# GadGadGad/Convolutional-KAN-for-Image-Classification

Measured on AMD Instinct MI355X. Metric: images/sec fwd+bwd KAN-VGG11 3x32x32 bs=256/GPU, higher is better.
Workload: dtype f32

## Files before the change

### convolutional-kan-for-image-classification_amd/_lib.py

```python
from __future__ import annotations

import ctypes as C
import os
from typing import Optional

_HERE = os.path.dirname(os.path.abspath(__file__))
LIB_PATH = os.environ.get("KANCONV_LIB") or os.path.join(_HERE, "libkanconv.so")

KAN_MAX_PLANES = 16
KAN_MAX_TABLE = 32
KAN_FP_WORDS = 192
BASIS_BSPLINE, BASIS_RBF, BASIS_CHEBY, BASIS_POLY, BASIS_FOURIER, BASIS_RELU, BASIS_GRAM = 0, 1, 2, 3, 4, 5, 6
ACT_NONE, ACT_IDENTITY, ACT_GELU, ACT_SILU, ACT_RELU, ACT_TANH, ACT_SIGMOID, ACT_GELU_TANH = -1, 0, 1, 2, 3, 4, 5, 6
ORDER_QUAD_FWD, ORDER_ROWBLK8_FWD, ORDER_QUAD_BWD_DATA, ORDER_FWD_WEIGHT_SIDE = 1, 2, 4, 8


class KanGeom(C.Structure):
    _fields_ = [(n, C.c_int) for n in ("B", "C", "H", "W", "O", "Ho", "Wo", "kh", "kw", "sh", "sw", "ph", "pw", "dh", "dw", "groups")] + \
               [("x_bstride", C.c_longlong), ("y_bstride", C.c_longlong)]


class KanBasis(C.Structure):
    _fields_ = [("kind", C.c_int), ("n_basis", C.c_int), ("order", C.c_int), ("act", C.c_int),
                ("p0", C.c_float), ("p1", C.c_float), ("table", C.c_float * KAN_MAX_TABLE), ("chan_table", C.c_void_p)]


class KanPlan(C.Structure):
    _fields_ = [(n, C.c_int) for n in ("P", "K", "IPC", "KC", "Kpad", "Opad", "fwd_splits", "bwd_data_splits", "bwd_weight_splits",
                                          "fwd_target", "bwd_data_target", "bwd_weight_target", "x_pm_wanted", "dz_pm_wanted", "bwd_weight_expanded", "row_blocks", "e_pm_wanted", "fwd_expanded", "fwd_halo", "bwd_weight_halo",
# ... 31 lines not shown
_GP, _BP = C.POINTER(KanGeom), C.POINTER(KanBasis)
SIGNATURES = {
    "kan_version": (C.c_char_p, []),
    "kan_last_error": (C.c_char_p, []),
    "kan_plan": (_I, [_GP, _BP, C.POINTER(KanPlan)]),
    "kan_tile_orders": (_I, [_GP, _BP]),
    "kan_pack_weights": (_I, [_P, _P, _P, _P, _GP, _BP, _P]),
    "kan_pack_weights_iod": (_I, [_P, _P, _P, _GP, _BP, _P]),
    "kan_pack_cacheable": (_I, [_GP, _BP]),
    "kan_pack_weights_cached": (_I, [_P, _P, _P, _P, _GP, _BP, _P, _I, _I, _I, _P]),
    "kan_conv_fwd": (_I, [_P, _P, _P, _P, _GP, _BP, _P, _P]),
    "kan_position_major": (_I, [_P, _P, _I, _I, _I, _LL, _P]),
    "kan_conv_bwd_data": (_I, [_P, _P, _P, _P, _P, _P, _GP, _BP, _P, _P]),
    "kan_conv_bwd_data_params": (_I, [_P, _P, _P, _P, _P, _P, _P, _GP, _BP, _P, _P]),
    "kan_conv_bwd_weight": (_I, [_P, _P, _P, _P, _GP, _BP, _P, _P, _P]),
    "kan_position_major_expanded": (_I, [_P, _P, _GP, _BP, _P]),
    "kan_conv_fwd_expanded": (_I, [_P, _P, _P, _GP, _BP, _P]),
    "kan_conv_fwd_expanded_order": (_I, [_P, _P, _P, _GP, _BP, _P, _I]),
    "kan_conv_bwd_weight_expanded": (_I, [_P, _P, _P, _GP, _BP, _P]),
    "kan_unpack_wgrad": (_I, [_P, _P, _P, _GP, _BP, _P]),
    "kan_unpack_wgrad_iod": (_I, [_P, _P, _GP, _BP, _P]),
    "kan_slab_reduce": (_I, [_P, _I, _LL, _P, _I, _I, _I, _LL, _P]),
    "kan_instnorm_prelu_fwd": (_I, [_P, _I, _LL, _P, _P, _P, _P, _P, _P, _P, _I, _I, _I, _LL, _F, _I, _P]),
    "kan_instnorm_prelu_bwd": (_I, [_P, _P, _P, _P, _P, _P, _P, _P, _P, _P, _P, _I, _I, _I, _LL, _I, _P]),
    "kan_instnorm_prelu_pool_fwd": (_I, [_P, _I, _LL, _P, _P, _P, _P, _P, _P, _P, _P, _I, _I, _I, _I, _LL, _F, _I, _P]),
    "kan_instnorm_prelu_pool_bwd": (_I, [_P, _P, _P, _P, _P, _P, _P, _P, _P, _P, _P, _P, _I, _I, _I, _I, _LL, _I, _P]),
    "kan_instnorm_prelu_poolk_fwd": (_I, [_P, _I, _LL, _P, _P, _P, _P, _P, _P, _P, _P, _I, _I, _I, _I, _LL, _F, _I, _I, _I, _P]),
    "kan_instnorm_prelu_poolk_bwd": (_I, [_P, _P, _P, _P, _P, _P, _P, _P, _P, _P, _P, _P, _I, _I, _I, _I, _LL, _I, _I, _I, _P]),
    "kan_norm_route": (_I, [_I, _I, _I, _I, _I, _LL, _I, _LL, _I, _I, _I, _I, C.POINTER(KanNormRoute)]),
    "kan_batchnorm_workspace_bytes": (_LL, [_I, _I]),
# ... 60 lines not shown
```

### convolutional-kan-for-image-classification_amd/csrc/kan_internal.h

```cpp
#pragma once
#include <type_traits>
#include "kanconv.h"

int kan_fail_msg(const char* fmt, const char* a);
int kan_raise_lds_limit(const void* kernel, int bytes);

enum : int {
    FAST_GENERIC = 0,
    FAST_BSPLINE_SILU = 1,
    FAST_BSPLINE_GELU = 2,
    FAST_RBF8 = 3,
    FAST_CHEBY5 = 4,
    FAST_CHEBY4 = 5,
    FAST_POLY4 = 6,
    FAST_POLY3 = 7,
    FAST_RBF5 = 8,
    FAST_RELU8 = 9,
    FAST_GRAM4 = 10,
    FAST_POLY1 = 11,
    FAST_LAST = 11
};
enum : unsigned {
    ON_TAP_MAJOR = 1u << 0,
    ON_BIG_TILES = 1u << 1,
// ... 93 lines not shown

struct FwdCfg { int TO, TP, tiles_o, tiles_p, chunks, splits, slots; };
struct BdCfg { int CH, tiles_c, tiles_p, n_ob, Opad32, chunks, splits; };
struct BwCfg { int TR, TO, tiles_r, tiles_o, chunks, splits, slots; };
struct BwHaloCfg { int R, nimg, spb, n_bands, tiles_r, tiles_o, splits, bands_per_split; };

struct ConvPlan {
    KanPlan pub;
    int fast;
    Route fwd, bwd_data, bwd_weight;
    bool pm_fwd, pm_bwd_data, pm_bwd_weight;
    bool rowblk_bwd_data;
    bool quad_fwd;
    bool quad_bd;
    bool rowblk8_fwd;
    bool fwd_wq;
    bool pmdma_xcd, pm_lpt, pm_xcd;
    FwdCfg fc;
    BdCfg bd;
    BwCfg bw;
    BwHaloCfg bwh;
    KanBandCfg band;
};
int plan_conv(const KanGeom* g, const KanBasis* b, ConvPlan* cp);

int live_taps_out(const KanGeom* g, int hw);
int live_taps_in(const KanGeom* g, int hw);
int live_positions_for_tap(const KanGeom* g, int tap);
int balance_tiles(const int* weight, int n, unsigned short* idx);
```

### convolutional-kan-for-image-classification_amd/csrc/kan_plan.hip

```cpp
#include <hip/hip_runtime.h>
#include <cstdio>
#include <cstdlib>
#include <cstring>
#include "kanconv.h"
#include "kan_device.h"
#include "kan_common.h"
#include "kan_internal.h"

namespace {

int fail(const char* msg) { return kan_fail_msg("%s", msg); }

int check(const KanGeom* g, const KanBasis* b) {
    if (!g || !b) return fail("null geometry/basis");
    if (g->groups < 0 || g->groups > 65535) return fail("groups out of range");
    if (g->B <= 0 || g->C <= 0 || g->O <= 0 || g->H <= 0 || g->W <= 0 || g->Ho <= 0 || g->Wo <= 0) return fail("non-positive dimension");
    if (g->kh <= 0 || g->kw <= 0 || g->sh <= 0 || g->sw <= 0 || g->dh <= 0 || g->dw <= 0 || g->ph < 0 || g->pw < 0) return fail("bad conv parameters");
    if (g->kh > 255 || g->kw > 255 || g->C > 65535) return fail("kernel size / channel count out of supported range");
    if ((g->H + 2 * g->ph - g->dh * (g->kh - 1) - 1) / g->sh + 1 != g->Ho || (g->W + 2 * g->pw - g->dw * (g->kw - 1) - 1) / g->sw + 1 != g->Wo)
        return fail("Ho/Wo inconsistent with H/W, kernel, stride, padding, dilation");
    if ((long long)g->B * g->Ho * g->Wo >= (1ll << 31) || (long long)g->B * g->H * g->W >= (1ll << 31)) return fail("pixel count exceeds int32");
    if ((long long)g->B * g->x_bstride * 4 >= (1ll << 31) || (long long)g->B * g->y_bstride * 4 >= (1ll << 31))
        return fail("activation tensors must be smaller than 2 GiB (32-bit buffer offsets)");
    if (g->x_bstride < (long long)ngroups(g) * g->C * g->H * g->W || g->y_bstride < (long long)ngroups(g) * g->O * g->Ho * g->Wo)
// ... 326 lines not shown
    c.fc = fwd_cfg(g, *pl, big, c.pm_fwd, halo);
    c.bw = bw_cfg(g, *pl, big, c.pm_bwd_weight);
    if (halo_bw) c.bwh = bw_halo_cfg(g, *pl);
    pl->fwd_splits = band ? c.band.fwd_splits : c.fc.splits;
    pl->bwd_data_splits = c.bd.splits;
    pl->bwd_weight_splits = halo_bw ? c.bwh.splits : c.bw.splits;
    if (band_bw) {
        pl->bwd_weight_splits = c.band.bw_splits;
        pl->bwd_weight_slab_elems = (long long)G * pl->Kpad * pl->Opad;
    }
    pl->fwd_target = pl->bwd_data_target = pl->bwd_weight_target = 0;
    const bool rowblk_fwd = halo && g->H == 4 && g->W == 4 && c.fc.TO == 256;
    c.quad_fwd = rowblk_fwd && g->B % 32 == 0 && !tuning_off("KAN_QUAD_FWD");
    c.quad_bd = c.rowblk_bwd_data && g->B % 32 == 0 && !tuning_off("KAN_QUAD_BD");
    c.rowblk8_fwd = halo && g->H == 8 && g->W == 8 && c.fc.TO == 256 && g->B % 4 == 0 && !tuning_off("KAN_ROWBLK8_FWD");
    c.fwd_wq = c.fwd == Route::EXPANDED && g->H == 2 && g->W == 2 && g->Ho == 2 && g->Wo == 2 && g->kh == 3 && g->kw == 3 && g->sh == 1 && g->sw == 1 &&
               g->ph == 1 && g->pw == 1 && g->dh == 1 && g->dw == 1 && pl->P == 9 && pl->KC == 18 && g->y_bstride % 4 == 0 && !tuning_off("KAN_PMDMA_FWD_WQ");
    if (dw) {
        pl->fwd_splits = pl->bwd_data_splits = 1;
        pl->bwd_weight_splits = dw_weight_chunks(g);
        pl->bwd_data_weight_bytes = pl->packed_weight_bytes;
        c.pm_fwd = c.pm_bwd_data = c.pm_bwd_weight = false;
    }
    if (c.pm_fwd) {
        LiveClass cls[16]; const int plane = g->Ho * g->Wo;
        const long long tiles_per_pos = (long long)ceil_div(g->B, c.fc.TP) * c.fc.tiles_o * G;
        for (int hw = 0; hw < plane; ++hw) cls[hw] = LiveClass{tiles_per_pos, live_taps_out(g, hw) * ceil_div(g->C, pl->IPC)};
        pl->fwd_target = pick_target_steps(cls, plane, 8, 4.0 * g->B * g->O * g->Ho * g->Wo * G, &pl->fwd_splits, c.fc.slots);
    }
    if (c.pm_bwd_weight) {
// ... 25 lines not shown
```

### convolutional-kan-for-image-classification_amd/csrc/kanconv.hip

```cpp
#include <hip/hip_runtime.h>
#include <cstdio>
#include <cstdlib>
#include <cstring>
#include <cmath>
#include <cstdint>
#include <mutex>
#include <type_traits>
#include <vector>
#include "kanconv.h"
#include "kan_device.h"

#include "kan_common.h"
#include "kan_internal.h"

namespace {


thread_local char g_err[512] = "";
int fail(const char* fmt, const char* a = "") {
    snprintf(g_err, sizeof(g_err), fmt, a);
    return -1;
}
}
int kan_fail_msg(const char* fmt, const char* a) { return fail(fmt, a); }
// ... 1296 lines not shown
        for (int r = 0; r < 16; ++r) {
            const int row = k0 + w_r * 64 + mi * 32 + mfma_row(r, lane);
            if (row >= Krows) continue;
#pragma unroll
            for (int ni = 0; ni < 2; ++ni) {
                const int o = o_tile0 + w_c * 64 + ni * 32 + (lane & 31);
                out[(size_t)row * Opad + o] = acc[mi][ni][r];
            }
        }
}

#define LDS_READ4W(r0, r1, r2, r3, a0, a1, b, oA, oB0, oB1)                                                              \
    asm volatile("ds_read_b32 %0, %4 offset:%7\n\tds_read_b32 %1, %5 offset:%7\n\tds_read_b32 %2, %6 offset:%8\n\tds_read_b32 %3, %6 offset:%9" \
                 : "=&v"(r0), "=&v"(r1), "=&v"(r2), "=&v"(r3) : "v"(a0), "v"(a1), "v"(b), "n"(oA), "n"(oB0), "n"(oB1) : "memory")

template <int FAST, int W, int R, int NIMG>
__global__ __launch_bounds__(256, 4) void k_conv_bwd_weight_halo(
    const float* __restrict__ dz, const float* __restrict__ x, float* __restrict__ dwp, DevGeom g, DevBasis bs, int Krows, int Opad,
    int n_bands, int bands_per_split, long long slab_elems, unsigned x_bytes, unsigned dz_bytes, int tiles_o) {
    constexpr int KIND = fast_kind(FAST);
    constexpr int P = fast_planes(FAST), T = 9, PT = P * T;
    constexpr int TR = 128, TO = 128, NT = 256, KPX = 16;
    constexpr int HWc = W + 2, HIMG = (R + 2) * HWc, CELLS = NIMG * HIMG;
    constexpr int PS = W == 16 ? CELLS + 1 : W == 8 ? CELLS + 3 : W == 4 ? CELLS + 7 : CELLS + 1;
    constexpr int NCH = (TR + PT - 2) / PT + 1;
    constexpr int HB = NCH * P * PS;
    constexpr int BP = NIMG * R * W, SPB = BP / KPX;
    constexpr int ZB = KPX * TO;
    constexpr int NU = NCH * NIMG * (R + 2) * W;
    constexpr int SLOTS = (NU + NT - 1) / NT;
    static_assert(BP % KPX == 0 && SPB % 2 == 0 && SPB >= SLOTS + 1 && PS > CELLS && (NIMG == 1 || R == W), "band shape");
    __shared__ float sH[2 * HB];
    __shared__ __attribute__((aligned(16))) float sZ[2 * ZB];
    __shared__ float sTab[KAN_MAX_TABLE];

    const int tid = threadIdx.x, lane = tid & 63;
    const int wave = __builtin_amdgcn_readfirstlane(tid >> 6);
    const int w_r = wave >> 1, w_c = wave & 1, kh2 = lane >> 5;
    const int HoWo = g.Ho * g.Wo, HW = g.H * g.W;
    const BlockId blk = xcd_block_order(true);
    const int grp = blk.y / tiles_o;
    const int k0 = blk.x * TR, o_tile0 = (blk.y - grp * tiles_o) * TO;
    x += (size_t)grp * g.C * HW;
    dz += (size_t)grp * g.O * HoWo;
    dwp += (size_t)grp * Krows * Opad;
    const int c0 = k0 / PT;

    if (tid < KAN_MAX_TABLE) sTab[tid] = bs.tab[tid];
    for (int i = tid; i < 2 * HB; i += NT) sH[i] = 0.f;
    float* const dump = sH + CELLS;

    int u_src[SLOTS], u_dst[SLOTS], u_hr[SLOTS], u_ch[SLOTS]; unsigned u_ok = 0;
#pragma unroll
    for (int k = 0; k < SLOTS; ++k) {
        const int idx = tid + k * NT;
        constexpr int UPC = NIMG * (R + 2) * W, UPI = (R + 2) * W;
        const int ch = idx / UPC, ri = idx - ch * UPC, img = ri / UPI, rc = ri - img * UPI, hr = rc / W, col = rc - hr * W;
        u_src[k] = (c0 + ch) * HW + img * (int)g.xbs + (hr - 1) * W + col;
        u_dst[k] = ch * (P * PS) + img * HIMG + hr * HWc + col + 1;
        u_hr[k] = hr - 1; u_ch[k] = c0 + ch;
        u_ok |= ((idx < NU && c0 + ch < g.C) ? 1u : 0u) << k;
    }
    const kan_rsrc x_rs = make_rsrc(x, x_bytes), dz_rs = make_rsrc(dz, dz_bytes);

    unsigned aA[2];
#pragma unroll
    for (int mi = 0; mi < 2; ++mi) {
        int row = k0 + w_r * 64 + mi * 32 + (lane & 31);
        if (row >= Krows) row = k0;
        const int c = row / PT, rem = row - c * PT, tap = rem / P, pl_ = rem - tap * P, r = tap / 3, t = tap - 3 * r;
        aA[mi] = lds_addr(sH + ((c - c0) * P + pl_) * PS + r * HWc + t + kh2);
    }
    unsigned bB[KPX / 2];
    {
        const int ol = w_c * 64 + (lane & 31), sw = (ol >> 1) & 15;
#pragma unroll
        for (int kk = 0; kk < KPX / 2; ++kk) bB[kk] = lds_addr(sZ + ol * KPX + ((2 * kk + kh2) ^ sw));
    }
    unsigned zoff[8];
#pragma unroll
    for (int j = 0; j < 8; ++j) {
        const int ol = 4 * (wave * 8 + j) + (lane >> 4), q = (lane & 15) ^ ((ol >> 1) & 15);
        zoff[j] = o_tile0 + ol < g.O ? (unsigned)((o_tile0 + ol) * HoWo + q) * 4u : KAN_OOB;
    }
    constexpr int BPI = NIMG > 1 ? 1 : (W * W) / BP;
    auto issue_dz = [&](int band, int st, int zb) {
        const int gpx = band * BP + st * KPX;
        const int b = gpx / (W * W), px0 = gpx - b * (W * W);
        const int soff = __builtin_amdgcn_readfirstlane((b * (int)g.ybs + px0) * 4);
        float* dst = sZ + zb * ZB + wave * (8 * 64);
#pragma unroll
        for (int j = 0; j < 8; ++j)
            __builtin_amdgcn_raw_ptr_buffer_load_lds(dz_rs, (__attribute__((address_space(3))) void*)(dst + j * 64), 4, (int)zoff[j], soff, 0, 0);
    };
    float xv[SLOTS]; unsigned inb_mask = 0;
    auto load_band = [&](int band) {
        const int b = NIMG > 1 ? band * NIMG : band / BPI, h0 = NIMG > 1 ? 0 : (band - b * BPI) * R;
        const int sbase = b * (int)g.xbs + h0 * W;
        inb_mask = 0;
#pragma unroll
        for (int k = 0; k < SLOTS; ++k) {
            const bool inb = ((u_ok >> k) & 1u) && (unsigned)(h0 + u_hr[k]) < (unsigned)g.H;
            xv[k] = buf_load(x_rs, inb ? (unsigned)(sbase + u_src[k]) * 4u : KAN_OOB);
            inb_mask |= (inb ? 1u : 0u) << k;
        }
// ... 22 lines not shown
    int hb = 0;
    for (int band = nb0; band < nb1; ++band, hb ^= 1) {
        const unsigned hoff = (unsigned)(hb * HB * 4);
        const unsigned a0 = aA[0] + hoff, a1 = aA[1] + hoff;
#pragma unroll
        for (int st = 0; st < SPB; ++st) {
            asm volatile("s_waitcnt vmcnt(0)" ::: "memory");
            __syncthreads();
            if (st + 1 < SPB) issue_dz(band, st + 1, (st + 1) & 1);
            else if (band + 1 < nb1) issue_dz(band + 1, 0, 0);
            if (st == 0) { if (band + 1 < nb1) load_band(band + 1); }
            else if (st - 1 < SLOTS) { if (band + 1 < nb1) expand(st - 1, hb ^ 1); }
            float fa[2][2], fb[2][2];
#define KAN_OFFA(kk) ((((16 * st + 2 * (kk)) / (R * W)) * HIMG + (((16 * st + 2 * (kk)) % (R * W)) / W) * HWc + ((16 * st + 2 * (kk)) % W)) * 4)
#define KAN_OFFB(kk) (((st & 1) * ZB) * 4)
            LDS_READ4W(fa[0][0], fa[0][1], fb[0][0], fb[0][1], a0, a1, bB[0], KAN_OFFA(0), KAN_OFFB(0), KAN_OFFB(0) + 32 * KPX * 4);
#pragma unroll
            for (int kk = 0; kk < KPX / 2; ++kk) {
                const int c_ = kk & 1, n_ = c_ ^ 1;
                if (kk + 1 < KPX / 2) {
                    LDS_READ4W(fa[n_][0], fa[n_][1], fb[n_][0], fb[n_][1], a0, a1, bB[kk + 1], KAN_OFFA(kk + 1), KAN_OFFB(kk + 1),
                               KAN_OFFB(kk + 1) + 32 * KPX * 4);
                    LDS_WAIT4(fa[c_][0], fa[c_][1], fb[c_][0], fb[c_][1], 4);
                } else {
                    LDS_WAIT4(fa[c_][0], fa[c_][1], fb[c_][0], fb[c_][1], 0);
                }
                acc[0][0] = MFMA32(fa[c_][0], fb[c_][0], acc[0][0]);
                acc[0][1] = MFMA32(fa[c_][0], fb[c_][1], acc[0][1]);
                acc[1][0] = MFMA32(fa[c_][1], fb[c_][0], acc[1][0]);
                acc[1][1] = MFMA32(fa[c_][1], fb[c_][1], acc[1][1]);
            }
#undef KAN_OFFA
#undef KAN_OFFB
        }
    }

    float* out = dwp + (size_t)blk.z * slab_elems;
#pragma unroll
    for (int mi = 0; mi < 2; ++mi)
#pragma unroll
        for (int r = 0; r < 16; ++r) {
            const int row = k0 + w_r * 64 + mi * 32 + mfma_row(r, lane);
            if (row >= Krows) continue;
#pragma unroll
            for (int ni = 0; ni < 2; ++ni) {
                const int o = o_tile0 + w_c * 64 + ni * 32 + (lane & 31);
                out[(size_t)row * Opad + o] = acc[mi][ni][r];
            }
        }
}

template <int KIND, int FAST>
__global__ __launch_bounds__(256) void k_expand_pm(const float* __restrict__ x, float* __restrict__ e_pm, DevBasis bs, int B, int CHW, int HW, int Cg,
                                                   long long bstride, float* __restrict__ dump) {
    __shared__ float tile[32][33];
    __shared__ float sTab[KAN_MAX_TABLE];
    const int e0 = blockIdx.x * 32, b0 = blockIdx.y * 32;
    const int tx = threadIdx.x & 31, ty = threadIdx.x >> 5;
// ... 1205 lines not shown

int kan_pack_weights(const float* w_base, const float* w_basis, float* wp, float* wd, const KanGeom* g, const KanBasis* b, void* stream) {
    return pack_weights_impl(w_base, w_basis, wp, wd, g, b, nullptr, 0, stream);
}

int kan_pack_weights_iod(const float* coeffs, float* wp, float* wd, const KanGeom* g, const KanBasis* b, void* stream) {
    if (int rc = iod_scope(g, b)) return rc;
    return pack_weights_impl(nullptr, coeffs, wp, wd, g, b, nullptr, 0, stream, true);
}

int kan_tile_orders(const KanGeom* g, const KanBasis* b) {
    ConvPlan cp;
    if (plan_conv(g, b, &cp)) return 0;
    const bool halo = cp.fwd == Route::HALO;
    return (halo && cp.quad_fwd ? KAN_ORDER_QUAD_FWD : 0) | (halo && cp.rowblk8_fwd ? KAN_ORDER_ROWBLK8_FWD : 0) | (cp.quad_bd ? KAN_ORDER_QUAD_BWD_DATA : 0) |
           (cp.fwd_wq ? KAN_ORDER_FWD_WEIGHT_SIDE : 0);
}

int kan_pack_cacheable(const KanGeom* g, const KanBasis* b) {
    ConvPlan cp;
    if (plan_conv(g, b, &cp)) return 0;
    if ((long long)g->O * g->C * (b->n_basis + 1) * g->kh * g->kw >= (1ll << 31)) return 0;
    return (!pack_needs_clear(g, cp.pub) && cp.fwd != Route::DW && ngroups(g) == 1) ? 1 : 0;
}

int kan_pack_weights_cached(const float* w_base, const float* w_basis, float* wp, float* wd, const KanGeom* g, const KanBasis* b,
                            unsigned long long* ring, int cur, int force, int sample_stride, void* stream) {
    static_assert(KAN_FP_WORDS == 3 * FP_LANES, "ring size");
    if (!ring || cur < 0 || cur > 2 || sample_stride < 1) return fail("bad fingerprint ring arguments");
    if (!kan_pack_cacheable(g, b)) return fail("cached packing is not offered for this geometry (kan_pack_cacheable)");
    const int hb = b->act != KAN_ACT_NONE;
// ... 200 lines not shown
                           decltype(rbv)::value == 2 ? dz_pm : dz, x, xn, wd,
                           dx, dxn, dg, db, c.CH, c.tiles_c, c.n_ob, c.Opad32, c.chunks, cps, pl.bwd_data_slab_elems, dz_bytes, perm, dpar);
    };
    const bool launched = dispatch_fast<ON_TAP_MAJOR>(fast, [&](auto fv) {
        constexpr int F = decltype(fv)::value;
        if constexpr (fast_has(F, ON_ROWBLK_BWD_DATA)) {
            if (quad) return launch(IC<fast_kind(F)>{}, fv, IC<2>{});
            if (rb) return launch(IC<fast_kind(F)>{}, fv, IC<1>{});
        }
        launch(IC<fast_kind(F)>{}, fv, IC<0>{});
    });
    if (!launched) dispatch_kind(b->kind, [&](auto kind) { launch(kind, IC<FAST_GENERIC>{}, IC<0>{}); });
    return launch_ok("conv_bwd_data");
}

int kan_conv_bwd_weight(const float* dz, const float* x, const float* xn, float* dwp, const KanGeom* g, const KanBasis* b,
                        const float* x_pm, const float* dz_pm, void* stream) {
    ConvPlan cp;
    if (int rc = plan_conv(g, b, &cp)) return rc;
    const KanPlan& pl = cp.pub;
    if (!dz || !x || !xn || !dwp) return fail("null tensor pointer");
    if ((b->kind == KAN_BASIS_RELU || b->kind == KAN_BASIS_GRAM) && !b->chan_table) return fail("ReLU / Gram bases need their device parameter table (chan_table)");
    hipStream_t st = (hipStream_t)stream;
    if (cp.bwd_weight == Route::DW) {
        DevGeom dgd = dev_geom(g); DevBasis dbd = dev_basis(b);
        dim3 grid(pl.bwd_weight_splits, ngroups(g));
        dispatch_kind(b->kind, [&](auto kind) {
            hipLaunchKernelGGL((k_dw_bwd_weight<decltype(kind)::value>), grid, dim3(256), 0, st, dz, x, xn, dwp, dgd, dbd, pl.K, pl.Opad, pl.bwd_weight_slab_elems);
        });
        return launch_ok("dw_bwd_weight");
    }
    if (cp.bwd_weight == Route::BAND) {
        if (x != xn && !fast_spec(cp.fast).xn_fwd) return fail("this basis / activation pair runs on single-input kernels: pass xn == x");
        return kan_band_bwd_weight_launch(dz, x, xn, dwp, g, b, &cp.band, pl.bwd_weight_splits, pl.bwd_weight_slab_elems, stream);
    }
    const unsigned x_bytes = (unsigned)((long long)g->B * g->x_bstride * 4), dz_bytes = (unsigned)((long long)g->B * g->y_bstride * 4);
    if (cp.bwd_weight == Route::HALO) {
        if (x != xn) return fail("internal: the channel-major weight-gradient layout needs x == xn");
        const BwHaloCfg& hc = cp.bwh;
        const DevGeom dgh = dev_geom(g); const DevBasis dbh = dev_basis(b);
        if ((long long)hc.tiles_o * ngroups(g) > 65535) return fail("groups * output tiles exceed the grid limit");
        dim3 grid(hc.tiles_r, hc.tiles_o * ngroups(g), hc.splits);
        dispatch_fast<ON_HALO_BWD_WEIGHT>(cp.fast, [&](auto fv) {
            auto launch = [&](auto w, auto r, auto nimg) {
                hipLaunchKernelGGL((k_conv_bwd_weight_halo<decltype(fv)::value, decltype(w)::value, decltype(r)::value, decltype(nimg)::value>), grid,
                                   dim3(256), 0, st, dz, x, dwp, dgh, dbh, pl.K, pl.Opad, hc.n_bands, hc.bands_per_split, pl.bwd_weight_slab_elems,
                                   x_bytes, dz_bytes, hc.tiles_o);
            };
            if (g->W == 16) launch(IC<16>{}, IC<4>{}, IC<1>{});
            else if (g->W == 8) launch(IC<8>{}, IC<8>{}, IC<1>{});
            else launch(IC<4>{}, IC<4>{}, IC<2>{});
        });
        return launch_ok("conv_bwd_weight_halo");
    }
    const BwCfg& c = cp.bw;
    DevGeom dg = dev_geom(g);
    dg.pix_major = (x_pm && dz_pm && x == xn && cp.pm_bwd_weight) ? 1 : 0;
    if (dg.pix_major) { x = x_pm; xn = x_pm; dz = dz_pm; }
    DevBasis db = dev_basis(b);
    if ((long long)c.tiles_o * ngroups(g) > 65535) return fail("groups * output tiles exceed the grid limit");
    dim3 grid(c.tiles_r, c.tiles_o * ngroups(g), pl.bwd_weight_splits);
    const int cps = dg.pix_major ? pl.bwd_weight_target : ceil_div(c.chunks, pl.bwd_weight_splits);
    if (x != xn && !fast_spec(cp.fast).xn_fwd)
        return fail("this basis / activation pair runs on single-input kernels: pass xn == x");
    auto launch = [&](auto kind, auto fast, auto wr, auto wc) {
        constexpr int WR = decltype(wr)::value, WC = decltype(wc)::value;
// ... 3 lines not shown
    auto tiles = [&](auto kind, auto fast) {
        if (c.TO == 128) launch(kind, fast, IC<2>{}, IC<2>{});
        else launch(kind, fast, IC<4>{}, IC<1>{});
    };
    const bool fast = dispatch_fast<ON_TAP_MAJOR>(cp.fast, [&](auto fv) {
        constexpr int F = decltype(fv)::value;
        if constexpr (fast_has(F, ON_BIG_TILES)) {
            if (c.TO == 256) return launch(IC<fast_kind(F)>{}, fv, IC<2>{}, IC<4>{});
        }
        tiles(IC<fast_kind(F)>{}, fv);
    });
    if (!fast) dispatch_kind(b->kind, [&](auto kind) { tiles(kind, IC<FAST_GENERIC>{}); });
    return launch_ok("conv_bwd_weight");
}

int kan_position_major_expanded(const float* x, float* e_pm, const KanGeom* g, const KanBasis* b, void* stream) {
    ConvPlan cp;
    if (int rc = plan_conv(g, b, &cp)) return rc;
    const KanPlan& pl = cp.pub;
    if (!x || !e_pm) return fail("null tensor pointer");
    if (!pl.e_pm_wanted) return fail("this geometry / basis does not use the expanded position-major copy (plan.e_pm_wanted)");
    const int G = ngroups(g), CHW = G * g->C * g->H * g->W;
    DevBasis db = dev_basis(b);
    dim3 grid(ceil_div(CHW, 32), ceil_div(g->B, 32));
    float* dump = e_pm + (pl.e_pm_elems - 256);
    if ((b->kind == KAN_BASIS_RELU || b->kind == KAN_BASIS_GRAM) && !b->chan_table) return fail("ReLU / Gram bases need their device parameter table (chan_table)");
    dispatch_fast<ON_EXPANDED>(cp.fast, [&](auto fv) {
        constexpr int F = decltype(fv)::value;
        hipLaunchKernelGGL((k_expand_pm<fast_kind(F), F>), grid, dim3(256), 0, (hipStream_t)stream, x, e_pm, db, g->B, CHW, g->H * g->W, g->C, g->x_bstride, dump);
    });
// ... 231 lines not shown
```

### convolutional-kan-for-image-classification_amd/ops.py

```python
from __future__ import annotations

import contextlib
import ctypes as C
import os
import weakref
from collections import OrderedDict
from dataclasses import dataclass, replace
from functools import lru_cache, partial
from typing import List, NamedTuple, Optional, Sequence, Tuple

import torch

from . import _lib as L


@dataclass(frozen=True)
class ConvSpec:
    kind: int
    n_basis: int
    order: int
    act: int
    p0: float
    p1: float
    table: Tuple[float, ...]
# ... 157 lines not shown
_ROW_BLOCK_BIT = {"fwd": 1, "bwd_data": 2, "bwd_weight": 0}


def _quadrant_order(geom, plan, which: str) -> bool:
    return which == "fwd" and bool(plan.row_blocks & 1) and geom.B % 32 == 0


def _quadrant_bwd_data(geom, plan, have_dz_pm: bool) -> bool:
    return bool(have_dz_pm) and bool(plan.row_blocks & 2) and bool(getattr(plan, "tile_orders", 0) & L.ORDER_QUAD_BWD_DATA)


def _row_blocks8_forward(geom, plan) -> bool:
    return geom.H == 8 and geom.W == 8 and bool(getattr(plan, "tile_orders", 0) & L.ORDER_ROWBLK8_FWD)


def _executed_flops(geom, plan, which: str, have_dz_pm: bool = False) -> float:
    target = {"fwd": plan.fwd_target, "bwd_data": plan.bwd_data_target, "bwd_weight": plan.bwd_weight_target}[which]
    dense = _conv_flops(geom, plan)
    g = geom
    if target <= 0:
        if _quadrant_order(geom, plan, which) or (which == "bwd_data" and _quadrant_bwd_data(geom, plan, have_dz_pm)):
            return dense * _live_fraction(which, g.H, g.W, g.Ho, g.Wo, g.kh, g.kw, g.sh, g.sw, g.ph, g.pw, g.dh, g.dw)
        if plan.row_blocks & _ROW_BLOCK_BIT[which]:
            return dense * (5.0 / 6.0)
        if which == "fwd" and _row_blocks8_forward(geom, plan):
            return dense * (11.0 / 12.0)
        return dense
    return dense * _live_fraction(which, g.H, g.W, g.Ho, g.Wo, g.kh, g.kw, g.sh, g.sw, g.ph, g.pw, g.dh, g.dw)


def _layer_tag(geom) -> str:
    return f"{geom.C * max(1, geom.groups)}->{geom.O * max(1, geom.groups)}@{geom.H}x{geom.W} k{geom.kh}x{geom.kw}"


def _sample(which: str, geom, plan, pm: bool, two: bool = False, expanded: bool = False):
    tile = "128" if plan.Opad % 128 == 0 else "64"
    if which == "bwd_data":
        name = "k_conv_bwd_data"
    elif expanded:
        name = f"k_conv_{which}_pmdma/o{tile}"
    elif plan.fwd_band if which == "fwd" else plan.bwd_weight_band:
        name = f"k_band_{which}/o" + ("128" if plan.Opad % 128 == 0 else "192" if plan.Opad == 192 else "64")
    else:
        halo = plan.fwd_halo if which == "fwd" else (plan.bwd_weight_halo and not two)
        name = f"k_conv_{which}{'_halo' if halo else ''}/o{tile}"
    skips = expanded or pm or bool(plan.row_blocks & _ROW_BLOCK_BIT[which]) or (which == "fwd" and _row_blocks8_forward(geom, plan))
    dense = _conv_flops(geom, plan)
    return name, dense, _executed_flops(geom, plan, which, pm) if skips else dense, _layer_tag(geom)


def _position_major(t: torch.Tensor, ch_off: int, Cn: int) -> torch.Tensor:
    B, Ct, H, W = t.shape
    out = torch.empty(Cn * H * W * B, device=t.device, dtype=torch.float32)
    L.check(L.load().kan_position_major(_ptr(t, ch_off * H * W), _ptr(out), B, Cn, H * W, Ct * H * W, _stream(t)), "kan_position_major")
    return out


def _stack(ws: Sequence[Optional[torch.Tensor]]) -> Optional[torch.Tensor]:
    if ws[0] is None:
        return None
    return ws[0].unsqueeze(0) if len(ws) == 1 else torch.stack(list(ws))
# ... 978 lines not shown
```

### include/kanconv.h

```cpp
#ifndef KANCONV_H
#define KANCONV_H

#ifdef __cplusplus
extern "C" {
#endif

#define KAN_MAX_PLANES 16
#define KAN_MAX_TABLE  32
#define KAN_FP_WORDS   192

enum { KAN_BASIS_BSPLINE = 0, KAN_BASIS_RBF = 1, KAN_BASIS_CHEBY = 2, KAN_BASIS_POLY = 3, KAN_BASIS_FOURIER = 4, KAN_BASIS_RELU = 5, KAN_BASIS_GRAM = 6 };
enum { KAN_ACT_NONE = -1, KAN_ACT_IDENTITY = 0, KAN_ACT_GELU = 1, KAN_ACT_SILU = 2, KAN_ACT_RELU = 3,
       KAN_ACT_TANH = 4, KAN_ACT_SIGMOID = 5, KAN_ACT_GELU_TANH = 6 };

typedef struct KanGeom {
    int B, C, H, W;
    int O, Ho, Wo;
    int kh, kw, sh, sw, ph, pw, dh, dw;
    int groups;
    long long x_bstride;
    long long y_bstride;
} KanGeom;

#define KAN_ORDER_PACK(mode, first) ((int)(mode) | ((int)(first) << 8))
// ... 26 lines not shown
    long long fwd_slab_elems;
    long long bwd_data_slab_elems;
    long long bwd_weight_slab_elems;
    long long e_pm_elems;
} KanPlan;

const char* kan_version(void);
const char* kan_last_error(void);

int kan_plan(const KanGeom* geom, const KanBasis* basis, KanPlan* plan);

#define KAN_ORDER_QUAD_FWD 1
#define KAN_ORDER_ROWBLK8_FWD 2
#define KAN_ORDER_QUAD_BWD_DATA 4
#define KAN_ORDER_FWD_WEIGHT_SIDE 8
int kan_tile_orders(const KanGeom* geom, const KanBasis* basis);

int kan_pack_weights(const float* w_base, const float* w_basis, float* wp, float* wd,
                     const KanGeom* geom, const KanBasis* basis, void* stream);

int kan_pack_weights_iod(const float* coeffs, float* wp, float* wd, const KanGeom* geom, const KanBasis* basis, void* stream);

int kan_pack_cacheable(const KanGeom* geom, const KanBasis* basis);
int kan_pack_weights_cached(const float* w_base, const float* w_basis, float* wp, float* wd,
                            const KanGeom* geom, const KanBasis* basis, unsigned long long* ring, int cur, int force,
                            int sample_stride, void* stream);

int kan_conv_fwd(const float* x, const float* xn, const float* wp, float* z,
                 const KanGeom* geom, const KanBasis* basis, const float* x_pm, void* stream);

int kan_position_major(const float* src, float* dst, int B, int Cn, int HW, long long bstride, void* stream);

int kan_conv_bwd_data(const float* dz, const float* x, const float* xn, const float* wd,
                      float* dx, float* dxn,
                      const KanGeom* geom, const KanBasis* basis, const float* dz_pm, void* stream);

int kan_conv_bwd_data_params(const float* dz, const float* x, const float* xn, const float* wd, float* dx, float* dxn, float* dparams,
                             const KanGeom* geom, const KanBasis* basis, const float* dz_pm, void* stream);

int kan_conv_bwd_weight(const float* dz, const float* x, const float* xn, float* dwp,
                        const KanGeom* geom, const KanBasis* basis, const float* x_pm, const float* dz_pm, void* stream);

int kan_position_major_expanded(const float* x, float* e_pm, const KanGeom* geom, const KanBasis* basis, void* stream);
int kan_conv_fwd_expanded(const float* e_pm, const float* wp, float* z, const KanGeom* geom, const KanBasis* basis, void* stream);
int kan_conv_fwd_expanded_order(const float* e_pm, const float* wp, float* z, const KanGeom* geom, const KanBasis* basis, void* stream, int order);
int kan_conv_bwd_weight_expanded(const float* dz_pm, const float* e_pm, float* dwp,
                                 const KanGeom* geom, const KanBasis* basis, void* stream);

int kan_unpack_wgrad(const float* dwp, float* dw_base, float* dw_basis,
                     const KanGeom* geom, const KanBasis* basis, void* stream);

int kan_unpack_wgrad_iod(const float* dwp, float* dcoeffs, const KanGeom* geom, const KanBasis* basis, void* stream);

int kan_slab_reduce(const float* slabs, int n_slabs, long long slab_elems, float* out,
                    int B, int Cn, int HW, long long bstride, void* stream);

// ... 115 lines not shown
```

Measured before the change: 18100.

## Add tap-row tiled halo weight-gradient kernel that skips dead halo rows

Adds a tap-row variant of the halo weight-gradient kernel for 8x8 and 16x16 planes with nine-plane bases. Each block handles one kernel row (split by blk.x % 3), stages only R rows without halo, and skips MFMA work and dz loads on the first or last band where that tap row falls in zero padding. It is on by default for W==8 and opt-in for W==16. The cost is a grid three times wider along K and twice as many bands, which means more blocks and more staging overhead per useful FLOP. An explicit order entry point and FLOP accounting in Python are also added.

```diff
diff --git a/convolutional-kan-for-image-classification_amd/_lib.py b/convolutional-kan-for-image-classification_amd/_lib.py
--- a/convolutional-kan-for-image-classification_amd/_lib.py
+++ b/convolutional-kan-for-image-classification_amd/_lib.py
@@ -12,7 +12,7 @@
 KAN_FP_WORDS = 192
 BASIS_BSPLINE, BASIS_RBF, BASIS_CHEBY, BASIS_POLY, BASIS_FOURIER, BASIS_RELU, BASIS_GRAM = 0, 1, 2, 3, 4, 5, 6
 ACT_NONE, ACT_IDENTITY, ACT_GELU, ACT_SILU, ACT_RELU, ACT_TANH, ACT_SIGMOID, ACT_GELU_TANH = -1, 0, 1, 2, 3, 4, 5, 6
-ORDER_QUAD_FWD, ORDER_ROWBLK8_FWD, ORDER_QUAD_BWD_DATA, ORDER_FWD_WEIGHT_SIDE = 1, 2, 4, 8
+ORDER_QUAD_FWD, ORDER_ROWBLK8_FWD, ORDER_QUAD_BWD_DATA, ORDER_FWD_WEIGHT_SIDE, ORDER_TAPROW_BWD_WEIGHT = 1, 2, 4, 8, 16
 
 
 class KanGeom(C.Structure):
@@ -74,6 +74,7 @@
     "kan_conv_bwd_data": (_I, [_P, _P, _P, _P, _P, _P, _GP, _BP, _P, _P]),
     "kan_conv_bwd_data_params": (_I, [_P, _P, _P, _P, _P, _P, _P, _GP, _BP, _P, _P]),
     "kan_conv_bwd_weight": (_I, [_P, _P, _P, _P, _GP, _BP, _P, _P, _P]),
+    "kan_conv_bwd_weight_order": (_I, [_P, _P, _P, _GP, _BP, _P, _I]),
     "kan_position_major_expanded": (_I, [_P, _P, _GP, _BP, _P]),
     "kan_conv_fwd_expanded": (_I, [_P, _P, _P, _GP, _BP, _P]),
     "kan_conv_fwd_expanded_order": (_I, [_P, _P, _P, _GP, _BP, _P, _I]),
diff --git a/convolutional-kan-for-image-classification_amd/csrc/kan_internal.h b/convolutional-kan-for-image-classification_amd/csrc/kan_internal.h
--- a/convolutional-kan-for-image-classification_amd/csrc/kan_internal.h
+++ b/convolutional-kan-for-image-classification_amd/csrc/kan_internal.h
@@ -131,6 +131,7 @@
     bool quad_fwd;
     bool quad_bd;
     bool rowblk8_fwd;
+    bool bw_taprow_ok, bw_taprow;
     bool fwd_wq;
     bool pmdma_xcd, pm_lpt, pm_xcd;
     FwdCfg fc;
diff --git a/convolutional-kan-for-image-classification_amd/csrc/kan_plan.hip b/convolutional-kan-for-image-classification_amd/csrc/kan_plan.hip
--- a/convolutional-kan-for-image-classification_amd/csrc/kan_plan.hip
+++ b/convolutional-kan-for-image-classification_amd/csrc/kan_plan.hip
@@ -364,6 +364,8 @@
     c.quad_fwd = rowblk_fwd && g->B % 32 == 0 && !tuning_off("KAN_QUAD_FWD");
     c.quad_bd = c.rowblk_bwd_data && g->B % 32 == 0 && !tuning_off("KAN_QUAD_BD");
     c.rowblk8_fwd = halo && g->H == 8 && g->W == 8 && c.fc.TO == 256 && g->B % 4 == 0 && !tuning_off("KAN_ROWBLK8_FWD");
+    c.bw_taprow_ok = c.bwd_weight == Route::HALO && (g->W == 8 || g->W == 16) && fast_planes(f) == 9;
+    c.bw_taprow = c.bw_taprow_ok && (g->W == 8 ? !tuning_off("KAN_BW_TAPROW") : tuning_on("KAN_BW_TAPROW"));
     c.fwd_wq = c.fwd == Route::EXPANDED && g->H == 2 && g->W == 2 && g->Ho == 2 && g->Wo == 2 && g->kh == 3 && g->kw == 3 && g->sh == 1 && g->sw == 1 &&
                g->ph == 1 && g->pw == 1 && g->dh == 1 && g->dw == 1 && pl->P == 9 && pl->KC == 18 && g->y_bstride % 4 == 0 && !tuning_off("KAN_PMDMA_FWD_WQ");
     if (dw) {
diff --git a/convolutional-kan-for-image-classification_amd/csrc/kanconv.hip b/convolutional-kan-for-image-classification_amd/csrc/kanconv.hip
--- a/convolutional-kan-for-image-classification_amd/csrc/kanconv.hip
+++ b/convolutional-kan-for-image-classification_amd/csrc/kanconv.hip
@@ -1334,22 +1334,25 @@
     asm volatile("ds_read_b32 %0, %4 offset:%7\n\tds_read_b32 %1, %5 offset:%7\n\tds_read_b32 %2, %6 offset:%8\n\tds_read_b32 %3, %6 offset:%9" \
                  : "=&v"(r0), "=&v"(r1), "=&v"(r2), "=&v"(r3) : "v"(a0), "v"(a1), "v"(b), "n"(oA), "n"(oB0), "n"(oB1) : "memory")
 
-template <int FAST, int W, int R, int NIMG>
+template <int FAST, int W, int R, int NIMG, int TRW = 0>
 __global__ __launch_bounds__(256, 4) void k_conv_bwd_weight_halo(
     const float* __restrict__ dz, const float* __restrict__ x, float* __restrict__ dwp, DevGeom g, DevBasis bs, int Krows, int Opad,
     int n_bands, int bands_per_split, long long slab_elems, unsigned x_bytes, unsigned dz_bytes, int tiles_o) {
     constexpr int KIND = fast_kind(FAST);
-    constexpr int P = fast_planes(FAST), T = 9, PT = P * T;
+    constexpr int P = fast_planes(FAST), T = 9, PT = P * T, PT3 = 3 * P;
     constexpr int TR = 128, TO = 128, NT = 256, KPX = 16;
-    constexpr int HWc = W + 2, HIMG = (R + 2) * HWc, CELLS = NIMG * HIMG;
-    constexpr int PS = W == 16 ? CELLS + 1 : W == 8 ? CELLS + 3 : W == 4 ? CELLS + 7 : CELLS + 1;
-    constexpr int NCH = (TR + PT - 2) / PT + 1;
+    constexpr int HR = TRW ? R : R + 2;
+    constexpr int HWc = W + 2, HIMG = HR * HWc, CELLS = NIMG * HIMG;
+    constexpr int PS = TRW ? CELLS + 1 : W == 16 ? CELLS + 1 : W == 8 ? CELLS + 3 : W == 4 ? CELLS + 7 : CELLS + 1;
+    constexpr int RT = TRW ? PT3 : PT;
+    constexpr int NCH = (TR + RT - 2) / RT + 1;
     constexpr int HB = NCH * P * PS;
     constexpr int BP = NIMG * R * W, SPB = BP / KPX;
     constexpr int ZB = KPX * TO;
-    constexpr int NU = NCH * NIMG * (R + 2) * W;
+    constexpr int NU = NCH * NIMG * HR * W;
     constexpr int SLOTS = (NU + NT - 1) / NT;
     static_assert(BP % KPX == 0 && SPB % 2 == 0 && SPB >= SLOTS + 1 && PS > CELLS && (NIMG == 1 || R == W), "band shape");
+    static_assert(!TRW || (NIMG == 1 && (W == 8 || W == 16) && W % R == 0), "tap-row tiles: 8x8 and 16x16 planes, bands inside one image");
     __shared__ float sH[2 * HB];
     __shared__ __attribute__((aligned(16))) float sZ[2 * ZB];
     __shared__ float sTab[KAN_MAX_TABLE];
@@ -1360,11 +1363,13 @@
     const int HoWo = g.Ho * g.Wo, HW = g.H * g.W;
     const BlockId blk = xcd_block_order(true);
     const int grp = blk.y / tiles_o;
-    const int k0 = blk.x * TR, o_tile0 = (blk.y - grp * tiles_o) * TO;
+    const int tr = TRW ? __builtin_amdgcn_readfirstlane(blk.x % 3) : 0;
+    const int k0 = (TRW ? blk.x / 3 : blk.x) * TR, o_tile0 = (blk.y - grp * tiles_o) * TO;
+    const int Klim = TRW ? Krows / 3 : Krows;
     x += (size_t)grp * g.C * HW;
     dz += (size_t)grp * g.O * HoWo;
     dwp += (size_t)grp * Krows * Opad;
-    const int c0 = k0 / PT;
+    const int c0 = k0 / RT;
 
     if (tid < KAN_MAX_TABLE) sTab[tid] = bs.tab[tid];
     for (int i = tid; i < 2 * HB; i += NT) sH[i] = 0.f;
@@ -1374,11 +1379,12 @@
 #pragma unroll
     for (int k = 0; k < SLOTS; ++k) {
         const int idx = tid + k * NT;
-        constexpr int UPC = NIMG * (R + 2) * W, UPI = (R + 2) * W;
+        constexpr int UPC = NIMG * HR * W, UPI = HR * W;
         const int ch = idx / UPC, ri = idx - ch * UPC, img = ri / UPI, rc = ri - img * UPI, hr = rc / W, col = rc - hr * W;
-        u_src[k] = (c0 + ch) * HW + img * (int)g.xbs + (hr - 1) * W + col;
+        const int sr = TRW ? hr + tr - 1 : hr - 1;
+        u_src[k] = (c0 + ch) * HW + img * (int)g.xbs + sr * W + col;
         u_dst[k] = ch * (P * PS) + img * HIMG + hr * HWc + col + 1;
-        u_hr[k] = hr - 1; u_ch[k] = c0 + ch;
+        u_hr[k] = sr; u_ch[k] = c0 + ch;
         u_ok |= ((idx < NU && c0 + ch < g.C) ? 1u : 0u) << k;
     }
     const kan_rsrc x_rs = make_rsrc(x, x_bytes), dz_rs = make_rsrc(dz, dz_bytes);
@@ -1387,8 +1393,8 @@
 #pragma unroll
     for (int mi = 0; mi < 2; ++mi) {
         int row = k0 + w_r * 64 + mi * 32 + (lane & 31);
-        if (row >= Krows) row = k0;
-        const int c = row / PT, rem = row - c * PT, tap = rem / P, pl_ = rem - tap * P, r = tap / 3, t = tap - 3 * r;
+        if (row >= Klim) row = k0;
+        const int c = row / RT, rem = row - c * RT, tap = rem / P, pl_ = rem - tap * P, r = TRW ? 0 : tap / 3, t = tap - 3 * r;
         aA[mi] = lds_addr(sH + ((c - c0) * P + pl_) * PS + r * HWc + t + kh2);
     }
     unsigned bB[KPX / 2];
@@ -1404,11 +1410,16 @@
         zoff[j] = o_tile0 + ol < g.O ? (unsigned)((o_tile0 + ol) * HoWo + q) * 4u : KAN_OOB;
     }
     constexpr int BPI = NIMG > 1 ? 1 : (W * W) / BP;
+    auto dead_first = [&](int band) { return TRW && tr == 0 && band % BPI == 0; };
+    auto dead_last = [&](int band) { return TRW && tr == 2 && band % BPI == BPI - 1; };
     auto issue_dz = [&](int band, int st, int zb) {
         const int gpx = band * BP + st * KPX;
         const int b = gpx / (W * W), px0 = gpx - b * (W * W);
         const int soff = __builtin_amdgcn_readfirstlane((b * (int)g.ybs + px0) * 4);
         float* dst = sZ + zb * ZB + wave * (8 * 64);
+        if constexpr (TRW != 0 && W == 16) {
+            if ((st == 0 && dead_first(band)) || (st == SPB - 1 && dead_last(band))) return;
+        }
 #pragma unroll
         for (int j = 0; j < 8; ++j)
             __builtin_amdgcn_raw_ptr_buffer_load_lds(dz_rs, (__attribute__((address_space(3))) void*)(dst + j * 64), 4, (int)zoff[j], soff, 0, 0);
@@ -1461,22 +1472,34 @@
             float fa[2][2], fb[2][2];
 #define KAN_OFFA(kk) ((((16 * st + 2 * (kk)) / (R * W)) * HIMG + (((16 * st + 2 * (kk)) % (R * W)) / W) * HWc + ((16 * st + 2 * (kk)) % W)) * 4)
 #define KAN_OFFB(kk) (((st & 1) * ZB) * 4)
-            LDS_READ4W(fa[0][0], fa[0][1], fb[0][0], fb[0][1], a0, a1, bB[0], KAN_OFFA(0), KAN_OFFB(0), KAN_OFFB(0) + 32 * KPX * 4);
-#pragma unroll
-            for (int kk = 0; kk < KPX / 2; ++kk) {
-                const int c_ = kk & 1, n_ = c_ ^ 1;
-                if (kk + 1 < KPX / 2) {
-                    LDS_READ4W(fa[n_][0], fa[n_][1], fb[n_][0], fb[n_][1], a0, a1, bB[kk + 1], KAN_OFFA(kk + 1), KAN_OFFB(kk + 1),
-                               KAN_OFFB(kk + 1) + 32 * KPX * 4);
-                    LDS_WAIT4(fa[c_][0], fa[c_][1], fb[c_][0], fb[c_][1], 4);
-                } else {
-                    LDS_WAIT4(fa[c_][0], fa[c_][1], fb[c_][0], fb[c_][1], 0);
-                }
-                acc[0][0] = MFMA32(fa[c_][0], fb[c_][0], acc[0][0]);
-                acc[0][1] = MFMA32(fa[c_][0], fb[c_][1], acc[0][1]);
-                acc[1][0] = MFMA32(fa[c_][1], fb[c_][0], acc[1][0]);
-                acc[1][1] = MFMA32(fa[c_][1], fb[c_][1], acc[1][1]);
-            }
+#define KAN_KPAIRS(K0, K1)                                                                                                                  \
+            {                                                                                                                               \
+                LDS_READ4W(fa[(K0) & 1][0], fa[(K0) & 1][1], fb[(K0) & 1][0], fb[(K0) & 1][1], a0, a1, bB[K0], KAN_OFFA(K0), KAN_OFFB(K0),  \
+                           KAN_OFFB(K0) + 32 * KPX * 4);                                                                                    \
+                _Pragma("unroll") for (int kk = (K0); kk < (K1); ++kk) {                                                                    \
+                    const int c_ = kk & 1, n_ = c_ ^ 1;                                                                                     \
+                    if (kk + 1 < (K1)) {                                                                                                    \
+                        LDS_READ4W(fa[n_][0], fa[n_][1], fb[n_][0], fb[n_][1], a0, a1, bB[kk + 1], KAN_OFFA(kk + 1), KAN_OFFB(kk + 1),      \
+                                   KAN_OFFB(kk + 1) + 32 * KPX * 4);                                                                        \
+                        LDS_WAIT4(fa[c_][0], fa[c_][1], fb[c_][0], fb[c_][1], 4);                                                           \
+                    } else {                                                                                                                \
+                        LDS_WAIT4(fa[c_][0], fa[c_][1], fb[c_][0], fb[c_][1], 0);                                                           \
+                    }                                                                                                                       \
+                    acc[0][0] = MFMA32(fa[c_][0], fb[c_][0], acc[0][0]);                                                                    \
+                    acc[0][1] = MFMA32(fa[c_][0], fb[c_][1], acc[0][1]);                                                                    \
+                    acc[1][0] = MFMA32(fa[c_][1], fb[c_][0], acc[1][0]);                                                                    \
+                    acc[1][1] = MFMA32(fa[c_][1], fb[c_][1], acc[1][1]);                                                                    \
+                }                                                                                                                           \
+            }
+            if constexpr (!TRW) {
+                KAN_KPAIRS(0, KPX / 2);
+            } else if constexpr (W == 16) {
+                if (!((st == 0 && dead_first(band)) || (st == SPB - 1 && dead_last(band)))) KAN_KPAIRS(0, KPX / 2);
+            } else {
+                if (!(st == 0 && dead_first(band))) KAN_KPAIRS(0, KPX / 4);
+                if (!(st == SPB - 1 && dead_last(band))) KAN_KPAIRS(KPX / 4, KPX / 2);
+            }
+#undef KAN_KPAIRS
 #undef KAN_OFFA
 #undef KAN_OFFB
         }
@@ -1487,8 +1510,9 @@
     for (int mi = 0; mi < 2; ++mi)
 #pragma unroll
         for (int r = 0; r < 16; ++r) {
-            const int row = k0 + w_r * 64 + mi * 32 + mfma_row(r, lane);
-            if (row >= Krows) continue;
+            int row = k0 + w_r * 64 + mi * 32 + mfma_row(r, lane);
+            if (row >= Klim) continue;
+            if constexpr (TRW != 0) { const int c = row / PT3; row += c * (PT - PT3) + tr * PT3; }
 #pragma unroll
             for (int ni = 0; ni < 2; ++ni) {
                 const int o = o_tile0 + w_c * 64 + ni * 32 + (lane & 31);
@@ -2724,7 +2748,7 @@
     if (plan_conv(g, b, &cp)) return 0;
     const bool halo = cp.fwd == Route::HALO;
     return (halo && cp.quad_fwd ? KAN_ORDER_QUAD_FWD : 0) | (halo && cp.rowblk8_fwd ? KAN_ORDER_ROWBLK8_FWD : 0) | (cp.quad_bd ? KAN_ORDER_QUAD_BWD_DATA : 0) |
-           (cp.fwd_wq ? KAN_ORDER_FWD_WEIGHT_SIDE : 0);
+           (cp.fwd_wq ? KAN_ORDER_FWD_WEIGHT_SIDE : 0) | (cp.bwd_weight == Route::HALO && cp.bw_taprow ? KAN_ORDER_TAPROW_BWD_WEIGHT : 0);
 }
 
 int kan_pack_cacheable(const KanGeom* g, const KanBasis* b) {
@@ -2955,12 +2979,15 @@
     return launch_ok("conv_bwd_data");
 }
 
-int kan_conv_bwd_weight(const float* dz, const float* x, const float* xn, float* dwp, const KanGeom* g, const KanBasis* b,
-                        const float* x_pm, const float* dz_pm, void* stream) {
+static int conv_bwd_weight_impl(const float* dz, const float* x, const float* xn, float* dwp, const KanGeom* g, const KanBasis* b,
+                                const float* x_pm, const float* dz_pm, void* stream, int order) {
     ConvPlan cp;
     if (int rc = plan_conv(g, b, &cp)) return rc;
     const KanPlan& pl = cp.pub;
     if (!dz || !x || !xn || !dwp) return fail("null tensor pointer");
+    if (order >= 0 && order != 0 && order != KAN_ORDER_TAPROW_BWD_WEIGHT) return fail("order must be 0 or KAN_ORDER_TAPROW_BWD_WEIGHT");
+    if (order >= 0 && cp.bwd_weight != Route::HALO) return fail("the weight gradient of this geometry / basis does not run the halo kernel (plan.bwd_weight_halo)");
+    if (order == KAN_ORDER_TAPROW_BWD_WEIGHT && !cp.bw_taprow_ok) return fail("this geometry does not offer the tap-row order (8x8 / 16x16 planes, nine-plane specs)");
     if ((b->kind == KAN_BASIS_RELU || b->kind == KAN_BASIS_GRAM) && !b->chan_table) return fail("ReLU / Gram bases need their device parameter table (chan_table)");
     hipStream_t st = (hipStream_t)stream;
     if (cp.bwd_weight == Route::DW) {
@@ -2981,16 +3008,23 @@
         const BwHaloCfg& hc = cp.bwh;
         const DevGeom dgh = dev_geom(g); const DevBasis dbh = dev_basis(b);
         if ((long long)hc.tiles_o * ngroups(g) > 65535) return fail("groups * output tiles exceed the grid limit");
-        dim3 grid(hc.tiles_r, hc.tiles_o * ngroups(g), hc.splits);
+        const bool taprow = order < 0 ? cp.bw_taprow : order != 0;
+        dim3 grid(taprow ? 3 * ceil_div(pl.K / 3, 128) : hc.tiles_r, hc.tiles_o * ngroups(g), hc.splits);
+        const int bmul = taprow ? 2 : 1;
         dispatch_fast<ON_HALO_BWD_WEIGHT>(cp.fast, [&](auto fv) {
-            auto launch = [&](auto w, auto r, auto nimg) {
-                hipLaunchKernelGGL((k_conv_bwd_weight_halo<decltype(fv)::value, decltype(w)::value, decltype(r)::value, decltype(nimg)::value>), grid,
-                                   dim3(256), 0, st, dz, x, dwp, dgh, dbh, pl.K, pl.Opad, hc.n_bands, hc.bands_per_split, pl.bwd_weight_slab_elems,
-                                   x_bytes, dz_bytes, hc.tiles_o);
+            auto launch = [&](auto w, auto r, auto nimg, auto trw) {
+                hipLaunchKernelGGL((k_conv_bwd_weight_halo<decltype(fv)::value, decltype(w)::value, decltype(r)::value, decltype(nimg)::value,
+                                                           decltype(trw)::value>), grid,
+                                   dim3(256), 0, st, dz, x, dwp, dgh, dbh, pl.K, pl.Opad, hc.n_bands * bmul, hc.bands_per_split * bmul,
+                                   pl.bwd_weight_slab_elems, x_bytes, dz_bytes, hc.tiles_o);
             };
-            if (g->W == 16) launch(IC<16>{}, IC<4>{}, IC<1>{});
-            else if (g->W == 8) launch(IC<8>{}, IC<8>{}, IC<1>{});
-            else launch(IC<4>{}, IC<4>{}, IC<2>{});
+            if constexpr (fast_planes(decltype(fv)::value) == 9) {
+                if (taprow && g->W == 16) return launch(IC<16>{}, IC<2>{}, IC<1>{}, IC<1>{});
+                if (taprow && g->W == 8) return launch(IC<8>{}, IC<4>{}, IC<1>{}, IC<1>{});
+            }
+            if (g->W == 16) launch(IC<16>{}, IC<4>{}, IC<1>{}, IC<0>{});
+            else if (g->W == 8) launch(IC<8>{}, IC<8>{}, IC<1>{}, IC<0>{});
+            else launch(IC<4>{}, IC<4>{}, IC<2>{}, IC<0>{});
         });
         return launch_ok("conv_bwd_weight_halo");
     }
@@ -3024,6 +3058,16 @@
     return launch_ok("conv_bwd_weight");
 }
 
+int kan_conv_bwd_weight(const float* dz, const float* x, const float* xn, float* dwp, const KanGeom* g, const KanBasis* b,
+                        const float* x_pm, const float* dz_pm, void* stream) {
+    return conv_bwd_weight_impl(dz, x, xn, dwp, g, b, x_pm, dz_pm, stream, -1);
+}
+
+int kan_conv_bwd_weight_order(const float* dz, const float* x, float* dwp, const KanGeom* g, const KanBasis* b, void* stream, int order) {
+    if (order < 0) return fail("order must be 0 or KAN_ORDER_TAPROW_BWD_WEIGHT");
+    return conv_bwd_weight_impl(dz, x, x, dwp, g, b, nullptr, nullptr, stream, order);
+}
+
 int kan_position_major_expanded(const float* x, float* e_pm, const KanGeom* g, const KanBasis* b, void* stream) {
     ConvPlan cp;
     if (int rc = plan_conv(g, b, &cp)) return rc;
diff --git a/convolutional-kan-for-image-classification_amd/ops.py b/convolutional-kan-for-image-classification_amd/ops.py
--- a/convolutional-kan-for-image-classification_amd/ops.py
+++ b/convolutional-kan-for-image-classification_amd/ops.py
@@ -195,6 +195,10 @@
     return geom.H == 8 and geom.W == 8 and bool(getattr(plan, "tile_orders", 0) & L.ORDER_ROWBLK8_FWD)
 
 
+def _tap_rows_bwd_weight(geom, plan) -> bool:
+    return bool(plan.bwd_weight_halo) and bool(getattr(plan, "tile_orders", 0) & L.ORDER_TAPROW_BWD_WEIGHT)
+
+
 def _executed_flops(geom, plan, which: str, have_dz_pm: bool = False) -> float:
     target = {"fwd": plan.fwd_target, "bwd_data": plan.bwd_data_target, "bwd_weight": plan.bwd_weight_target}[which]
     dense = _conv_flops(geom, plan)
@@ -206,6 +210,8 @@
             return dense * (5.0 / 6.0)
         if which == "fwd" and _row_blocks8_forward(geom, plan):
             return dense * (11.0 / 12.0)
+        if which == "bwd_weight" and _tap_rows_bwd_weight(geom, plan):
+            return dense * (1.0 - 2.0 / (3.0 * g.H))
         return dense
     return dense * _live_fraction(which, g.H, g.W, g.Ho, g.Wo, g.kh, g.kw, g.sh, g.sw, g.ph, g.pw, g.dh, g.dw)
 
@@ -225,7 +231,8 @@
     else:
         halo = plan.fwd_halo if which == "fwd" else (plan.bwd_weight_halo and not two)
         name = f"k_conv_{which}{'_halo' if halo else ''}/o{tile}"
-    skips = expanded or pm or bool(plan.row_blocks & _ROW_BLOCK_BIT[which]) or (which == "fwd" and _row_blocks8_forward(geom, plan))
+    skips = expanded or pm or bool(plan.row_blocks & _ROW_BLOCK_BIT[which]) or (which == "fwd" and _row_blocks8_forward(geom, plan)) or \
+        (which == "bwd_weight" and not two and _tap_rows_bwd_weight(geom, plan))
     dense = _conv_flops(geom, plan)
     return name, dense, _executed_flops(geom, plan, which, pm) if skips else dense, _layer_tag(geom)
 
diff --git a/include/kanconv.h b/include/kanconv.h
--- a/include/kanconv.h
+++ b/include/kanconv.h
@@ -64,6 +64,7 @@
 #define KAN_ORDER_ROWBLK8_FWD 2
 #define KAN_ORDER_QUAD_BWD_DATA 4
 #define KAN_ORDER_FWD_WEIGHT_SIDE 8
+#define KAN_ORDER_TAPROW_BWD_WEIGHT 16
 int kan_tile_orders(const KanGeom* geom, const KanBasis* basis);
 
 int kan_pack_weights(const float* w_base, const float* w_basis, float* wp, float* wd,
@@ -90,6 +91,7 @@
 
 int kan_conv_bwd_weight(const float* dz, const float* x, const float* xn, float* dwp,
                         const KanGeom* geom, const KanBasis* basis, const float* x_pm, const float* dz_pm, void* stream);
+int kan_conv_bwd_weight_order(const float* dz, const float* x, float* dwp, const KanGeom* geom, const KanBasis* basis, void* stream, int order);
 
 int kan_position_major_expanded(const float* x, float* e_pm, const KanGeom* geom, const KanBasis* basis, void* stream);
 int kan_conv_fwd_expanded(const float* e_pm, const float* wp, float* z, const KanGeom* geom, const KanBasis* basis, void* stream);
```

Result: no change. 18150, median of 6 (+0.3%).
